# huang-yh/SelfOcc

Hardware: AMD Instinct MI355X
Metric: rendered rays/sec (6-cam 450x800, 128 samples/ray) (higher is better)
Workload: dtype f32; 1 GPU; BASELINE configs[1]: 6 cams x 450x800 rays, 128 samples/ray, volume 200x200x16; volume_channels=1, feat_storage=f32, preheat_steps=150

## Files before the change

### selfocc_amd/csrc/render_fwd.hip

```cpp
#include "render_row.h"
#include "ray_device.h"

int so_render_fwd_samples(const so_render_args &a, hipStream_t st);

namespace {

SO_DEVFN RayGeom so_pixel_ray(const so_render_args &a, int cam, int ix, int iy) {
    typedef const __attribute__((address_space(4))) float *so_const_fptr;
    const so_const_fptr M = (so_const_fptr)(a.img2lidar + cam * 16);
    float u = (float)ix * a.sx + a.ox;
    float v = (float)iy * a.sy + a.oy;
    RayGeom g;
    g.ox = M[3]; g.oy = M[7]; g.oz = M[11];
    float dx = (M[0] * u + M[1] * v) + M[2];
    float dy = (M[4] * u + M[5] * v) + M[6];
    float dz = (M[8] * u + M[9] * v) + M[10];
    g.dn = sqrtf((dx * dx + dy * dy) + dz * dz);
    g.dx = dx / g.dn; g.dy = dy / g.dn; g.dz = dz / g.dn;
    return g;
}

template <int NF, bool BF16>
SO_DEVFN void so_gather_feat(const void *__restrict__ vol, int H, int W, int D, const so_cell &c,
                             const float wk[8], float f[NF > 0 ? NF : 1]) {
// ... 781 lines not shown
        st.gh = gh; st.gw = gw; st.gd = gd;
        const int h0 = so_floor_i(gh), w0 = so_floor_i(gw), d0 = so_floor_i(gd);
        st.h0 = h0; st.w0 = w0; st.d0 = d0;
        st.cell = so_cell_index(h0, w0, d0, W, D);
    };
    auto interior = [&](const AheadStep &st) __attribute__((always_inline)) {
        return so_all3((unsigned)st.h0 < (unsigned)(H - 1), (unsigned)st.w0 < (unsigned)(W - 1), (unsigned)st.d0 < (unsigned)(D - 1));
    };
    int i_lo = S, i_hi = -1;
    {
        AheadStep p;
        const int n = min(kSureScan, S);
#pragma nounroll
        for (int k = 0; k < n; ++k) {
            place(k, p);
            if (interior(p)) { i_lo = k; break; }
        }
        if (i_lo < S) {
#pragma nounroll
            for (int k = S - 1; k >= S - n && k >= i_lo; --k) {
                place(k, p);
                if (interior(p)) { i_hi = k; break; }
            }
        }
        if (i_hi < 0) i_lo = S;
    }
    auto locate = [&](const int i, AheadStep &st, auto in_sure) __attribute__((always_inline)) {
        place(i, st);
        if constexpr (decltype(in_sure)::value) {
            st.code = __builtin_amdgcn_raw_buffer_load_b8(rb, st.cell, codes_off, 0);
        } else {
            st.all_interior = interior(st);
            st.code = 0u;
            if (st.all_interior) st.code = __builtin_amdgcn_raw_buffer_load_b8(rb, st.cell, codes_off, 0);
        }
    };
    auto near_face = [&](float fh, float fw, float fd) __attribute__((always_inline)) {
        return fmaxf(fmaxf(fabsf(fh - 0.5f), fabsf(fw - 0.5f)), fabsf(fd - 0.5f)) > 0.5f - face_m;
    };
    auto canon_cell = [&](const int i) __attribute__((always_inline)) {
        RayGeom gc = geom(so_reload_args());
        {
            unsigned ones = ~0u;
            asm volatile("" : "+s"(ones));
            const unsigned lane = __builtin_amdgcn_mbcnt_hi(ones, __builtin_amdgcn_mbcnt_lo(ones, 0u));
            const float *slot = s_dir + (wave_slot + lane);
            gc.dx = slot[0]; gc.dy = slot[256]; gc.dz = slot[512];
        }
        __builtin_amdgcn_sched_barrier(0);
        float px, py, pz;
        {
            const so_render_args ac = so_reload_args();
            const int n = ac.n_samples;
            const float b0 = so_bin(i, n);
            const float t_start = b0 * tfar + (1.0f - b0) * tnear;
            if (ac.sample_pos == SO_SAMPLE_AT_START) {
                px = gc.ox + gc.dx * t_start; py = gc.oy + gc.dy * t_start; pz = gc.oz + gc.dz * t_start;
            } else {
                const float b1 = so_bin(i + 1, n);
                const float tt = t_start + (b1 * tfar + (1.0f - b1) * tnear);
                px = gc.ox + (gc.dx * tt) / 2.0f; py = gc.oy + (gc.dy * tt) / 2.0f; pz = gc.oz + (gc.dz * tt) / 2.0f;
            }
        }
        __builtin_amdgcn_sched_barrier(0);
        float slope;
        auto axis = [](so_axis A) __attribute__((always_inline)) { A.size1 = 0.0f; return A; };
        const float gh = so_grid_coord(so_axis_m2g(axis(so_reload_args().map.h), py, slope), so_reload_args().map.h.tot_len);
        __builtin_amdgcn_sched_barrier(0);
        const float gw = so_grid_coord(so_axis_m2g(axis(so_reload_args().map.w), px, slope), so_reload_args().map.w.tot_len);
        __builtin_amdgcn_sched_barrier(0);
        const float gd = so_grid_coord(so_axis_m2g(axis(so_reload_args().map.d), pz, slope), so_reload_args().map.d.tot_len);
        return so_cell_of(gh, gw, gd);
    };

    auto step = [&](const int i, AheadStep &cur, AheadStep &nxt, auto in_sure, bool &hint) __attribute__((always_inline)) {
        constexpr bool IN_SURE = decltype(in_sure)::value;
        bool skip;
        if constexpr (IN_SURE) {
            const auto free_lanes = __builtin_amdgcn_ballot_w64((int)cur.code >= rcode);
            skip = free_lanes == __builtin_amdgcn_ballot_w64(true);
            if constexpr (kLowMode) hint = free_lanes == 0;
            locate(i + 1, nxt, in_sure);
        } else {
            skip = cur.all_interior && so_all((int)cur.code >= rcode);
            if (i + 1 < S) locate(i + 1, nxt, in_sure);
        }
        float w;
        if (skip) {
            w = kAlphaFree * T;
            T = T * ((1.0f - kAlphaFree) + 1e-7f);
        } else {
            float fh = __builtin_amdgcn_fractf(cur.gh), fw = __builtin_amdgcn_fractf(cur.gw), fd = __builtin_amdgcn_fractf(cur.gd);
            so_f32x2 p0, p1, p2, p3;
            auto gather = [&](int h0, int w0, int d0) __attribute__((always_inline)) {
                float v[8];
                so_gather_sdf_buf(rs, H, W, D, h0, w0, d0, v);
                p0 = so_f32x2{v[0], v[4]}; p1 = so_f32x2{v[1], v[5]}; p2 = so_f32x2{v[2], v[6]}; p3 = so_f32x2{v[3], v[7]};
            };
            bool moved_any = false;
            if (FACE_SAFE && __builtin_expect(__any(near_face(fh, fw, fd)), 0)) {
                int h0 = cur.h0, w0 = cur.w0, d0 = cur.d0;
                bool moved = false;
                if (near_face(fh, fw, fd)) {
                    const so_cell c = canon_cell(i);
                    moved = (c.h0 != h0) | (c.w0 != w0) | (c.d0 != d0);
                    h0 = moved ? c.h0 : h0; w0 = moved ? c.w0 : w0; d0 = moved ? c.d0 : d0;
                    fh = moved ? c.fh1 : fh; fw = moved ? c.fw1 : fw; fd = moved ? c.fd1 : fd;
                }
                moved_any = __any(moved);
                if (moved_any) gather(h0, w0, d0);
            }
            if (__builtin_expect(!moved_any, 1)) {
                if (IN_SURE || cur.all_interior) {
                    {
                        const so_f4v lo = so_bload4(rb, cur.cell * 16u, 0u), hi = so_bload4(rb, cur.cell * 16u, row_off);
                        p0 = lo.xy; p1 = lo.zw; p2 = hi.xy; p3 = hi.zw;
                    }
                } else {
                    gather(cur.h0, cur.w0, cur.d0);
                }
            }
            float sdf, dh0, gvw, gvd;
            so_trilerp_fast_pk(p0, p1, p2, p3, fh, fw, fd, sdf, dh0, gvw, gvd);
            const float cosv = fmaf(gvd, Gdd, fmaf(gvw, Gdw, dh0 * Gdh));
            const float alpha = so_alpha_fast(sdf * s2, fminf(cosv, 0.0f) * hdt_s2);
            w = alpha * T;
            T = T * ((1.0f - alpha) + 1e-7f);
        }
        const float t_mid = fmaf(cur.fi, dt, tnear + hdt);
        acc = acc + w;
        dsum = fmaf(w, t_mid, dsum);
        if (w > best_w) { best_w = w; best_t = t_mid; }
        return skip;
    };

    auto low = [&](int &i, AheadStep &st) __attribute__((always_inline)) {
        struct so_f3 { float h, w, d; };
        using so_f3r = so_f3 &;
        auto fractions = [&]() __attribute__((always_inline)) {
            return so_f3{__builtin_amdgcn_fractf(st.gh), __builtin_amdgcn_fractf(st.gw), __builtin_amdgcn_fractf(st.gd)};
        };
        so_f3 f0 = fractions(), f1;
        bool coded = false;
        bool go = i + 1 < i_hi && !(FACE_SAFE && __any(near_face(f0.h, f0.w, f0.d)));
        auto trip = [&](so_f4v &lo, so_f4v &hi, so_f4v &nlo, so_f4v &nhi, so_f3r f, so_f3r nf) __attribute__((always_inline)) {
            if constexpr (!kLowPrefetch) { lo = so_bload4(rb, st.cell * 16u, 0u); hi = so_bload4(rb, st.cell * 16u, row_off); }
            float t_mid = fmaf(st.fi, dt, tnear + hdt);
            asm volatile("" : "+v"(t_mid));
            ++i;
            place(i, st);
            if constexpr (kLowPrefetch) {
                nlo = so_bload4(rb, st.cell * 16u, 0u); nhi = so_bload4(rb, st.cell * 16u, row_off);
                __builtin_amdgcn_sched_barrier(0);
                nf = fractions();
            }
            const bool proven = __any(lo.x <= low_thr);
            float sdf, dh0, gvw, gvd;
            so_trilerp_fast_pk(lo.xy, lo.zw, hi.xy, hi.zw, f.h, f.w, f.d, sdf, dh0, gvw, gvd);
            const float cosv = fmaf(gvd, Gdd, fmaf(gvw, Gdw, dh0 * Gdh));
            float alpha = so_alpha_fast(sdf * s2, fminf(cosv, 0.0f) * hdt_s2);
            if (__builtin_expect(!proven, 0)) {
                AheadStep was;
                place(i - 1, was);
                const unsigned code = __builtin_amdgcn_raw_buffer_load_b8(rb, was.cell, codes_off, 0);
                unsigned next_cell = st.cell;
                if constexpr (kLowPrefetch) {
                    int ia = i;
                    asm volatile("" : "+s"(ia));
                    AheadStep now;
                    place(ia, now);
                    next_cell = now.cell;
                }
                st.code = __builtin_amdgcn_raw_buffer_load_b8(rb, next_cell, codes_off, 0);
                if (so_all((int)code >= rcode)) alpha = kAlphaFree;
                coded = true;
            }
            const float w = alpha * T;
            T = T * ((1.0f - alpha) + 1e-7f);
            acc = acc + w;
            dsum = fmaf(w, t_mid, dsum);
            if (w > best_w) { best_w = w; best_t = t_mid; }
            if constexpr (!kLowPrefetch) nf = fractions();
            go = !coded && !over_now() && i + 1 < i_hi && !(FACE_SAFE && __any(near_face(nf.h, nf.w, nf.d)));
        };
        so_f4v lo0, hi0, lo1, hi1;
        if constexpr (kLowPrefetch) {
            if (go) {
                lo0 = so_bload4(rb, st.cell * 16u, 0u); hi0 = so_bload4(rb, st.cell * 16u, row_off);
#pragma nounroll
                for (;;) {
                    trip(lo0, hi0, lo1, hi1, f0, f1);
                    if (!go) break;
                    trip(lo1, hi1, lo0, hi0, f1, f0);
                    if (!go) break;
                }
                int ii = i;
                asm volatile("" : "+s"(ii));
                place(ii, st);
            }
        } else {
#pragma nounroll
            while (go) trip(lo0, hi0, lo1, hi1, f0, f0);
        }
        if (over_now()) return true;
        if (!coded) st.code = __builtin_amdgcn_raw_buffer_load_b8(rb, st.cell, codes_off, 0);
        return false;
    };

    auto run = [&](int &i, AheadStep &st) __attribute__((always_inline)) {
        auto free_step = [&]() __attribute__((always_inline)) {
            const float t_mid = fmaf(st.fi, dt, tnear + hdt);
            ++i;
            place(i, st);
            st.code = __builtin_amdgcn_raw_buffer_load_b8(rb, st.cell, codes_off, 0);
            const float w = kAlphaFree * T;
            T = T * ((1.0f - kAlphaFree) + 1e-7f);
            acc = acc + w;
            dsum = fmaf(w, t_mid, dsum);
        };
        const bool kept = kSpentExit ? (__builtin_amdgcn_ballot_w64(T * 0x1p24f >= acc) & __builtin_amdgcn_ballot_w64(T >= 2e-10f)) != 0
                                     : !so_all(T < 2e-10f);
        if (S <= kRunExitFreeSteps && kept) {
            while (i < i_hi && so_all((int)st.code >= rcode)) free_step();
        } else {
            while (i < i_hi && so_all((int)st.code >= rcode)) {
                free_step();
                if (over_now()) return true;
            }
        }
        return false;
    };

    {
        constexpr std::false_type general{};
        constexpr std::true_type in_sure{};
        AheadStep A, B;
        locate(0, A, general);
        int i = 0;
        bool over = false, unused_hint = false;
        auto gen = [&](int end) __attribute__((always_inline)) {
#pragma nounroll
            while (i < end) {
                step(i, A, B, general, unused_hint);
                if (++i >= S || over_now()) { over = true; break; }
                A = B;
            }
        };
        gen(i_lo);
        if (!over) {
            while (i < i_hi) {
                const bool sa = step(i, A, B, in_sure, low_hint_a);
                ++i;
                if (over_now() || (sa && run(i, B))) { over = true; break; }
                if (i >= i_hi) { A = B; break; }
                const bool sb = step(i, B, A, in_sure, low_hint_b);
                ++i;
                if (over_now() || (sb && run(i, A))) { over = true; break; }
                if constexpr (kLowMode) {
                    if (low_hint_a && low_hint_b && low(i, A)) { over = true; break; }
                }
            }
            if (!over) { A.all_interior = true; gen(S); }
        }
    }

    const float eps32 = 1.1920928955078125e-07f;
    if (dt * inv_dn < eps32) best_t = tnear + hdt;
    float depth = dsum * so_fast_rcp(acc + 1e-10f);
    if (a.flags & SO_FLAG_DEPTH_DIV_NORM) depth = depth * inv_dn;
    if (a.depth) a.depth[ray] = depth;
    if (a.acc) a.acc[ray] = acc;
    if (a.max_depth) a.max_depth[ray] = best_t * inv_dn;
    if (a.nears) a.nears[ray] = tnear;
    if (a.fars) a.fars[ray] = tfar;
}

enum class March {
    Canonical,
    Fast,
    FastFaceSafe,
    Skip,
    SkipFaceSafe,
    CanonicalUpscale,
};
constexpr bool so_is_fast(March m) { return m == March::Fast || m == March::FastFaceSafe; }
constexpr bool so_is_skip(March m) { return m == March::Skip || m == March::SkipFaceSafe; }
constexpr bool so_face_safe(March m) { return m == March::FastFaceSafe || m == March::SkipFaceSafe; }
template <class ROW>
constexpr bool so_is_staged(March m) { return so_is_fast(m) && !ROW::BF16 && ROW::NF >= 4; }

template <class ROW, March MODE, class GeomFn>
SO_DEVFN void so_march(const so_render_args &a, int ray, GeomFn geom) {
    static_assert(!so_is_skip(MODE), "skip marcher: the kernels that take so_launch_consts");
    if constexpr (MODE == March::CanonicalUpscale) {
        so_march_exact<ROW, SO_MAP_UPSCALE>(a, ray, geom(a));
    } else if constexpr (so_is_fast(MODE)) {
        so_march_fast<ROW, false, so_face_safe(MODE)>(a, ray, geom);
    } else {
        so_march_exact<ROW, SO_MAP_LINEAR>(a, ray, geom(a));
    }
}


__global__ __launch_bounds__(256) void sdf_brickify_kernel(const float *__restrict__ vol, float *__restrict__ brick,
                                                           int H, int W, int D, so_render_args a, int with_codes,
                                                           so_launch_consts c) {
    const int h = blockIdx.x, h1 = min(h + 1, H - 1);
    const size_t n_cells = (size_t)H * W * D;
    uint8_t *codes = (uint8_t *)(brick + n_cells * 4);
    const bool quads = (D & 3) == 0 && (blockDim.x & 3) == 0;
    const float kd = c.kd.k1, kw = c.kw.k1, kh = c.kh.k1;
    for (int w = blockIdx.y * blockDim.y + threadIdx.y; w < W; w += gridDim.y * blockDim.y) {
        const int w1 = min(w + 1, W - 1);
        const float *r00 = vol + ((size_t)h * W + w) * D, *r01 = vol + ((size_t)h * W + w1) * D;
        const float *r10 = vol + ((size_t)h1 * W + w) * D, *r11 = vol + ((size_t)h1 * W + w1) * D;
        for (int d = threadIdx.x; d < D; d += blockDim.x) {
            const int d1 = min(d + 1, D - 1);
            const float v0 = r00[d], v1 = r00[d1], v2 = r01[d], v3 = r01[d1];
            const float v4 = r10[d], v5 = r10[d1], v6 = r11[d], v7 = r11[d1];
            const size_t cell = ((size_t)h * W + w) * D + d;
            ((float4 *)brick)[cell] = make_float4(v0, v4, v1, v5);
            unsigned code = 0u;
            if (with_codes) {
                const float m = fminf(fminf(fminf(v0, v1), fminf(v2, v3)), fminf(fminf(v4, v5), fminf(v6, v7)));
                const float gd = fmaxf(fmaxf(fabsf(v1 - v0), fabsf(v3 - v2)), fmaxf(fabsf(v5 - v4), fabsf(v7 - v6))) * kd;
                const float gw = fmaxf(fmaxf(fabsf(v2 - v0), fabsf(v3 - v1)), fmaxf(fabsf(v6 - v4), fabsf(v7 - v5))) * kw;
                const float gh = fmaxf(fmaxf(fabsf(v4 - v0), fabsf(v5 - v1)), fmaxf(fabsf(v6 - v2), fabsf(v7 - v3))) * kh;
                const float G = sqrtf((gd * gd + gw * gw) + gh * gh) * 1.001f + 1e-20f;
                const float slack = m - kSkipArg / so_inv_s(a);
                if (slack > 0.0f && so_inv_s(a) > 0.0f) {
                    const float allow = 2.0f * slack / G / c.skip_unit;
                    code = (unsigned)fminf(floorf(allow * 0.999f), 255.0f);
                }
            }
            if (quads) {
                const unsigned c1 = (unsigned)__builtin_amdgcn_update_dpp(0, (int)code, 0x55, 0xf, 0xf, false);
                const unsigned c2 = (unsigned)__builtin_amdgcn_update_dpp(0, (int)code, 0xaa, 0xf, 0xf, false);
                const unsigned c3 = (unsigned)__builtin_amdgcn_update_dpp(0, (int)code, 0xff, 0xf, 0xf, false);
                if ((d & 3) == 0) *(unsigned *)(codes + cell) = code | (c1 << 8) | (c2 << 16) | (c3 << 24);
            } else {
                codes[cell] = (uint8_t)code;
            }
        }
    }
}

struct TilePixel { int cam, ix, iy, wave, lane; };
SO_DEVFN TilePixel so_tile_pixel(int tiles_x, int tiles_y) {
    const int b = blockIdx.x;
    const int cam = b / (tiles_x * tiles_y);
    const int tb = b - cam * tiles_x * tiles_y;
    const int ty = tb / tiles_x, tx = tb - ty * tiles_x;
    const int wave = threadIdx.x >> 6, lane = threadIdx.x & 63;
    return {cam, tx * 16 + (wave & 1) * 8 + (lane & 7), ty * 16 + (wave >> 1) * 8 + (lane >> 3), wave, lane};
}

template <class ROW>
constexpr int so_min_blocks() { return (ROW::NB == 0 && ROW::NF >= 8) ? 2 : 1; }

template <class ROW, March MODE>
__global__ __launch_bounds__(256, so_min_blocks<ROW>()) void render_fwd_explicit(so_render_args a) {
    int ray = blockIdx.x * blockDim.x + threadIdx.x;
    if (ray >= a.n_rays) return;
    auto geom = [&](const so_render_args &a) __attribute__((always_inline)) { return so_explicit_ray(a, ray); };
    so_march<ROW, MODE>(a, ray, geom);
}

template <class ROW, March MODE>
SO_DEVFN void pixgrid_body(const so_render_args &a, int tiles_x, int tiles_y) {
    const TilePixel p = so_tile_pixel(tiles_x, tiles_y);
    const int cam = p.cam, wave = p.wave, lane = p.lane;
    int ix = p.ix, iy = p.iy;
    if constexpr (so_is_staged<ROW>(MODE)) {
        constexpr int NF = ROW::NF;
        __shared__ __attribute__((aligned(16))) float s_stage[4 * StageGeom<NF>::kWaveDwords];
        const bool real = (ix < a.nx) && (iy < a.ny);
        ix = min(ix, a.nx - 1); iy = min(iy, a.ny - 1);
        int ray = (cam * a.ny + iy) * a.nx + ix;
        auto geom = [&](const so_render_args &a) __attribute__((always_inline)) { return so_pixel_ray(a, cam, ix, iy); };
        constexpr int NSEM_LDS = NF - 3 >= 16 ? NF - 3 : 0;
        __shared__ float s_sem[NSEM_LDS > 0 ? NSEM_LDS * 256 : 1];
        so_march_fast<ROW, true, so_face_safe(MODE)>(a, ray, geom, real, s_stage + wave * StageGeom<NF>::kWaveDwords, lane,
                                                     s_sem + threadIdx.x);
    } else {
        if (ix >= a.nx || iy >= a.ny) return;
        int ray = (cam * a.ny + iy) * a.nx + ix;
        auto geom = [&](const so_render_args &a) __attribute__((always_inline)) { return so_pixel_ray(a, cam, ix, iy); };
        so_march<ROW, MODE>(a, ray, geom);
    }
}

template <class ROW, March MODE>
__global__ __launch_bounds__(256, so_min_blocks<ROW>()) void render_fwd_pixgrid(so_render_args a, int tiles_x, int tiles_y) {
    if constexpr (ROW::NB > 0) {
        const int b = blockIdx.x;
        const int cam = b / (tiles_x * tiles_y);
        const int tb = b - cam * tiles_x * tiles_y;
        const int ty = tb / tiles_x, tx = tb - ty * tiles_x;
        const int wave = threadIdx.x >> 6, lane = threadIdx.x & 63;
        const int ix = tx * 16 + (wave & 1) * 8 + (lane & 7);
        const int iy = ty * 16 + (wave >> 1) * 8 + (lane >> 3);
        if (ix >= a.nx || iy >= a.ny) return;
        const int ray = (cam * a.ny + iy) * a.nx + ix;
        so_march_exact<ROW, MODE == March::CanonicalUpscale ? SO_MAP_UPSCALE : SO_MAP_LINEAR>(a, ray, so_pixel_ray(a, cam, ix, iy));
    } else {
        pixgrid_body<ROW, MODE>(a, tiles_x, tiles_y);
    }
}

template <class ROW, March MODE>
__global__ __launch_bounds__(256, 1) void render_fwd_explicit(so_render_args a, so_launch_consts c) {
    static_assert(so_is_skip(MODE) && ROW::NF == 0 && ROW::NB == 0, "skip marcher: SDF-only launches");
    int ray = blockIdx.x * blockDim.x + threadIdx.x;
    if (ray >= a.n_rays) return;
    auto geom = [&](const so_render_args &a) __attribute__((always_inline)) { return so_explicit_ray(a, ray); };
    so_march_fast_ahead<so_face_safe(MODE)>(a, c, ray, geom);
}
#ifdef SO_NO_ROW_ORDER
constexpr bool kRowsOutermost = false;
#else
constexpr bool kRowsOutermost = true;
#endif
template <class ROW, March MODE>
__global__ __launch_bounds__(256, 1) __attribute__((amdgpu_num_sgpr(80))) void render_fwd_pixgrid(so_render_args a, so_launch_consts c) {
    static_assert(so_is_skip(MODE) && ROW::NF == 0 && ROW::NB == 0, "skip marcher: SDF-only launches");
    const int cam = kRowsOutermost ? blockIdx.y : blockIdx.z, row = kRowsOutermost ? blockIdx.z : blockIdx.y;
    const int wave = threadIdx.x >> 6, lane = threadIdx.x & 63;
    const int ix = blockIdx.x * 16 + (wave & 1) * 8 + (lane & 7), iy = row * 16 + (wave >> 1) * 8 + (lane >> 3);
    if (ix >= a.nx || iy >= a.ny) return;
    const int ray = (cam * a.ny + iy) * a.nx + ix;
    auto geom = [&](const so_render_args &a) __attribute__((always_inline)) { return so_pixel_ray(a, cam, ix, iy); };
    so_march_fast_ahead<so_face_safe(MODE)>(a, c, ray, geom);
}
bool so_skip_grid_fits(const so_render_args &a) {
    return a.ray_mode == SO_RAYS_EXPLICIT || ((a.ny + 15) / 16 <= 65535 && a.n_cams <= 65535);
}

template <class ROW, March MODE>
int launch_fwd(const so_render_args &a, hipStream_t st) {
    const int tiles_x = (a.nx + 15) / 16, tiles_y = (a.ny + 15) / 16;
    if constexpr (so_is_skip(MODE)) {
        const so_launch_consts c = so_make_launch_consts(a);
        if (a.ray_mode == SO_RAYS_EXPLICIT) {
            hipLaunchKernelGGL((render_fwd_explicit<ROW, MODE>), dim3((a.n_rays + 255) / 256), dim3(256), 0, st, a, c);
        } else {
            const dim3 grid = kRowsOutermost ? dim3(tiles_x, a.n_cams, tiles_y) : dim3(tiles_x, tiles_y, a.n_cams);
            hipLaunchKernelGGL((render_fwd_pixgrid<ROW, MODE>), grid, dim3(256), 0, st, a, c);
        }
    } else if (a.ray_mode == SO_RAYS_EXPLICIT) {
        int blocks = (a.n_rays + 255) / 256;
        hipLaunchKernelGGL((render_fwd_explicit<ROW, MODE>), dim3(blocks), dim3(256), 0, st, a);
    } else {
        int blocks = tiles_x * tiles_y * a.n_cams;
        hipLaunchKernelGGL((render_fwd_pixgrid<ROW, MODE>), dim3(blocks), dim3(256), 0, st, a, tiles_x, tiles_y);
    }
    return so_launch_status();
}

void so_launch_brickify(const so_render_args &a, hipStream_t st, int with_codes) {
    const int H = a.map.h.tot_len, W = a.map.w.tot_len, D = a.map.d.tot_len;
    int qx = 1;
    while (qx < D && qx < 256) qx *= 2;
    const int wy = 256 / qx;
    hipLaunchKernelGGL(sdf_brickify_kernel, dim3(H, min((W + wy - 1) / wy, 65535)), dim3(qx, wy), 0, st, a.sdf_vol, a.sdf_brick,
                       H, W, D, a, with_codes, so_make_launch_consts(a));
}

bool so_fast_eligible(const so_render_args &a) {
    return !(a.flags & SO_FLAG_EXACT) && a.jitter_mode == SO_JITTER_NONE && a.map.kind == SO_MAP_LINEAR &&
           a.map.h.size1 == 0.0f && a.map.w.size1 == 0.0f && a.map.d.size1 == 0.0f &&
           (long long)a.map.h.tot_len * a.map.w.tot_len < (1 << 24) && a.map.d.tot_len < (1 << 24);
}

template <class ROW, int MK>
int dispatch(const so_render_args &a, hipStream_t st) {
    if constexpr (MK == SO_MAP_UPSCALE) return launch_fwd<ROW, March::CanonicalUpscale>(a, st);
    else if constexpr (ROW::NB > 0) return launch_fwd<ROW, March::Canonical>(a, st);
    else {
        if (!so_fast_eligible(a)) return launch_fwd<ROW, March::Canonical>(a, st);
        constexpr bool CAN_SKIP = ROW::NF == 0;
        if (a.sdf_brick) so_launch_brickify(a, st, (CAN_SKIP && !(a.flags & SO_FLAG_NO_SKIP)) ? 1 : 0);
        const bool face_safe = ROW::MASKED || !(a.flags & SO_FLAG_NO_FACE_SAFE);
        if constexpr (CAN_SKIP) {
            if (a.sdf_brick && !(a.flags & (SO_FLAG_NO_SKIP | SO_FLAG_NO_AHEAD)) && so_skip_grid_fits(a))
                return face_safe ? launch_fwd<ROW, March::SkipFaceSafe>(a, st) : launch_fwd<ROW, March::Skip>(a, st);
        }
        if constexpr (!ROW::MASKED) {
            if (!face_safe) return launch_fwd<ROW, March::Fast>(a, st);
        }
        return launch_fwd<ROW, March::FastFaceSafe>(a, st);
    }
}

}

int so_validate_mapping(const so_mapping &m) {
    SO_REQUIRE(m.kind == SO_MAP_LINEAR || m.kind == SO_MAP_UPSCALE, "mapping: unknown kind %d (0 = linear, 1 = linear_upscale)",
               (int)m.kind);
    const so_axis *ax[3] = {&m.h, &m.w, &m.d};
    const so_upscale_axis *ux[3] = {&m.uh, &m.uw, &m.ud};
    for (int i = 0; i < 3; ++i) {
        SO_REQUIRE(ax[i]->tot_len >= 2, "mapping axis %d: tot_len must be >= 2", i);
        SO_REQUIRE(ax[i]->size0 > 0 && ax[i]->range0 > 0, "mapping axis %d: size0/range0 must be > 0", i);
        if (m.kind == SO_MAP_LINEAR) {
            SO_REQUIRE(ax[i]->size1 == 0 || ax[i]->range1 > 0, "mapping axis %d: range1 must be > 0", i);
        } else {
            SO_REQUIRE(ax[i]->size1 >= 1, "linear_upscale axis %d: outer cells must be >= 1 (got %g)", i, (double)ax[i]->size1);
            SO_REQUIRE(ux[i]->unit > 0 && __builtin_isfinite(ux[i]->unit), "linear_upscale axis %d: unit must be > 0 (got %g)", i,
                       (double)ux[i]->unit);
            SO_REQUIRE(ux[i]->inc > 0 && __builtin_isfinite(ux[i]->inc),
                       "linear_upscale axis %d: increase unit must be > 0 (got %g): the outer range must exceed outer * unit",
                       i, (double)ux[i]->inc);
        }
    }
    return 0;
}

namespace {
template <int MK>
__global__ __launch_bounds__(256) void meter2grid_kernel(so_mapping m, const float *__restrict__ xyz, int n, int normalize,
                                                         float *__restrict__ hwd) {
    const int i = blockIdx.x * blockDim.x + threadIdx.x;
    if (i >= n) return;
    float gh, gw, gd, sh, sw, sd;
    so_m2g<MK>(m, xyz[3 * (size_t)i], xyz[3 * (size_t)i + 1], xyz[3 * (size_t)i + 2], gh, gw, gd, sh, sw, sd);
    if (normalize) {
        gh = gh / (float)(m.h.tot_len - 1); gw = gw / (float)(m.w.tot_len - 1); gd = gd / (float)(m.d.tot_len - 1);
    }
    hwd[3 * (size_t)i] = gh; hwd[3 * (size_t)i + 1] = gw; hwd[3 * (size_t)i + 2] = gd;
}
}

extern "C" int selfocc_meter2grid(const so_mapping *map, const float *xyz, int n, int normalize, float *hwd, void *stream) {
    SO_REQUIRE(map != nullptr, "map is NULL");
    if (so_validate_mapping(*map)) return -1;
    SO_REQUIRE(n >= 0, "n must be >= 0");
    if (n == 0) return 0;
    SO_REQUIRE(xyz != nullptr && hwd != nullptr, "xyz / hwd is NULL");
    const dim3 grid((unsigned)((n + 255) / 256));
    if (map->kind == SO_MAP_UPSCALE)
        hipLaunchKernelGGL(meter2grid_kernel<SO_MAP_UPSCALE>, grid, dim3(256), 0, (hipStream_t)stream, *map, xyz, n, normalize, hwd);
    else
        hipLaunchKernelGGL(meter2grid_kernel<SO_MAP_LINEAR>, grid, dim3(256), 0, (hipStream_t)stream, *map, xyz, n, normalize, hwd);
    return so_launch_status();
}

int so_validate_render(const so_render_args &a) {
    if (so_validate_mapping(a.map)) return -1;
    SO_REQUIRE(a.sdf_vol != nullptr, "sdf_vol is NULL");
    SO_REQUIRE(a.n_samples >= 1, "n_samples must be >= 1");
    SO_REQUIRE(a.n_rays >= 0, "n_rays must be >= 0");
    SO_REQUIRE(a.n_rgb == 0 || a.n_rgb == 3, "n_rgb must be 0 or 3 (the colour outputs; sh_deg sets the coefficient count)");
    SO_REQUIRE(a.n_sem >= 0, "n_sem must be >= 0");
    SO_REQUIRE(a.n_sem == 0 || a.n_rgb == 3, "semantic channels require n_rgb == 3");
    SO_REQUIRE(a.sh_deg >= 0 && a.sh_deg <= 2, "sh_deg %d is not built (built: sh_deg 0, 1, 2)", (int)a.sh_deg);
    SO_REQUIRE(a.sh_act == SO_SH_RELU || a.sh_act == SO_SH_SIGMOID, "sh_act %d is unknown (0 = relu, 1 = sigmoid)", (int)a.sh_act);
    if (a.n_rgb + a.n_sem > 0) {
        SO_REQUIRE(a.feat_vol != nullptr, "feat_vol is NULL but n_rgb + n_sem > 0");
        SO_REQUIRE(a.feat_dtype == SO_DTYPE_F32 || a.feat_dtype == SO_DTYPE_BF16, "bad feat_dtype");
        SO_REQUIRE(a.feat_stride % 4 == 0 && a.feat_stride >= a.n_rgb + a.n_sem,
                   "feat_stride must be a multiple of 4 and >= n_rgb + n_sem");
    }
    if (so_sh_launch(a)) {
        const int n_coef = 3 * (a.sh_deg + 1) * (a.sh_deg + 1);
        SO_REQUIRE(a.n_sem == 0, "sh_deg > 0 / sh_act = sigmoid with n_sem = %d semantic channels is not built (built: n_sem = 0)",
                   (int)a.n_sem);
        SO_REQUIRE(a.feat_dtype == SO_DTYPE_F32, "sh_deg > 0 / sh_act = sigmoid with a bfloat16 feature volume is not built (built: float32)");
        SO_REQUIRE(a.feat_stride == so_sh_stride(n_coef / 3), "sh_deg = %d reads %d coefficients: feat_stride must be %d (got %d)",
                   (int)a.sh_deg, n_coef, so_sh_stride(n_coef / 3), (int)a.feat_stride);
    }
    if (a.n_sem > 0 && !so_sh_launch(a)) {
        const int stride = so_row_width(a.n_sem);
        SO_REQUIRE(a.n_sem != 1, "n_sem = 1 is not built (built: n_sem 0 and 2 .. 21): one class renders `acc`");
        SO_REQUIRE(a.n_sem <= 21, "n_sem = %d is not built (built: n_sem 0 and 2 .. 21): the binned backward record and the "
                   "32-lanes-per-sample brick kernel end at 24 channels", (int)a.n_sem);
        SO_REQUIRE(a.feat_stride == stride, "n_sem = %d semantic channels: feat_stride must be %d = 3 + n_sem rounded up to 4 (got %d)",
                   (int)a.n_sem, stride, (int)a.feat_stride);
        SO_REQUIRE(a.feat_dtype == SO_DTYPE_F32 || a.n_sem == 21, "bfloat16 feature volumes with semantic channels are built for "
                   "n_sem = 21, feat_stride = 24 only (got n_sem = %d)", (int)a.n_sem);
    }
    if (a.ray_mode == SO_RAYS_EXPLICIT) {
        SO_REQUIRE(a.n_rays == 0 || (a.origins && a.dirs), "explicit rays need origins and dirs");
    } else if (a.ray_mode == SO_RAYS_PIXEL_GRID) {
        SO_REQUIRE(a.img2lidar != nullptr, "pixel-grid rays need img2lidar");
        SO_REQUIRE(a.n_cams >= 0 && a.nx >= 0 && a.ny >= 0, "bad pixel grid");
        SO_REQUIRE((int64_t)a.n_cams * a.nx * a.ny == a.n_rays, "n_rays != n_cams * ny * nx");
    } else {
        SO_REQUIRE(false, "bad ray_mode %d", a.ray_mode);
    }
    SO_REQUIRE(a.jitter_mode >= SO_JITTER_NONE && a.jitter_mode <= SO_JITTER_EDGES, "bad jitter_mode %d", (int)a.jitter_mode);
    SO_REQUIRE(a.jitter_mode == SO_JITTER_NONE || a.t_rand, "jitter or explicit edges requested but t_rand is NULL");
    SO_REQUIRE(a.bkgd_mode != SO_BKGD_PER_RAY || a.bkgd_rays, "per-ray background but bkgd_rays is NULL");
    SO_REQUIRE(a.sample_pos == SO_SAMPLE_AT_START || a.sample_pos == SO_SAMPLE_AT_MID, "bad sample_pos");
    return 0;
}

extern "C" int selfocc_render_fwd(const so_render_args *args, void *stream) {
    SO_REQUIRE(args != nullptr, "args is NULL");
    const so_render_args &a = *args;
    if (so_validate_render(a)) return -1;
    if (a.n_rays == 0) return 0;
    hipStream_t st = (hipStream_t)stream;
    if (a.weights || a.ts || a.deltas || a.sdf || a.grad) return so_render_fwd_samples(a, st);
    return so_with_row_and_map(a, [&](auto row, auto mk) { return dispatch<decltype(row), decltype(mk)::value>(a, st); });
}
```

Baseline: 8.146 billion rays/s.

## Process two H slices per brickify thread, reusing rows via buffer loads

```diff
diff --git a/selfocc_amd/csrc/render_fwd.hip b/selfocc_amd/csrc/render_fwd.hip
--- a/selfocc_amd/csrc/render_fwd.hip
+++ b/selfocc_amd/csrc/render_fwd.hip
@@ -1107,44 +1107,71 @@
 }
 
 
+constexpr int kBrickHB = 2;
+constexpr int kBrickRecordAux = 16;
+SO_DEVFN float so_bload1(__amdgpu_buffer_rsrc_t r, unsigned voff, unsigned soff) {
+    return __builtin_bit_cast(float, __builtin_amdgcn_raw_buffer_load_b32(r, voff, soff, 0));
+}
+struct so_brick_row { float v00, v01, v10, v11; };
+SO_DEVFN so_brick_row so_brick_load_row(__amdgpu_buffer_rsrc_t rv, unsigned o00, unsigned o01, unsigned o10, unsigned o11,
+                                        unsigned row) {
+    return {so_bload1(rv, o00, row), so_bload1(rv, o01, row), so_bload1(rv, o10, row), so_bload1(rv, o11, row)};
+}
 __global__ __launch_bounds__(256) void sdf_brickify_kernel(const float *__restrict__ vol, float *__restrict__ brick,
                                                            int H, int W, int D, so_render_args a, int with_codes,
                                                            so_launch_consts c) {
-    const int h = blockIdx.x, h1 = min(h + 1, H - 1);
-    const size_t n_cells = (size_t)H * W * D;
-    uint8_t *codes = (uint8_t *)(brick + n_cells * 4);
+    typedef unsigned so_u4v __attribute__((ext_vector_type(4)));
+    const int h_lo = blockIdx.x * kBrickHB, h_hi = min(h_lo + kBrickHB, H);
+    const __amdgpu_buffer_rsrc_t rv = so_make_rsrc(vol, (size_t)c.n_cells * 4);
+    const __amdgpu_buffer_rsrc_t rb = so_make_rsrc(brick, (size_t)c.n_cells * 17);
+    const unsigned slice = (unsigned)W * (unsigned)D;
     const bool quads = (D & 3) == 0 && (blockDim.x & 3) == 0;
     const float kd = c.kd.k1, kw = c.kw.k1, kh = c.kh.k1;
+    const float inv_s = so_inv_s(a);
+    const float sat = kSkipArg / inv_s;
+    const bool can_skip = with_codes && inv_s > 0.0f;
     for (int w = blockIdx.y * blockDim.y + threadIdx.y; w < W; w += gridDim.y * blockDim.y) {
         const int w1 = min(w + 1, W - 1);
-        const float *r00 = vol + ((size_t)h * W + w) * D, *r01 = vol + ((size_t)h * W + w1) * D;
-        const float *r10 = vol + ((size_t)h1 * W + w) * D, *r11 = vol + ((size_t)h1 * W + w1) * D;
+        const unsigned c0 = __umul24((unsigned)w, (unsigned)D), c1 = __umul24((unsigned)w1, (unsigned)D);
         for (int d = threadIdx.x; d < D; d += blockDim.x) {
             const int d1 = min(d + 1, D - 1);
-            const float v0 = r00[d], v1 = r00[d1], v2 = r01[d], v3 = r01[d1];
-            const float v4 = r10[d], v5 = r10[d1], v6 = r11[d], v7 = r11[d1];
-            const size_t cell = ((size_t)h * W + w) * D + d;
-            ((float4 *)brick)[cell] = make_float4(v0, v4, v1, v5);
-            unsigned code = 0u;
-            if (with_codes) {
-                const float m = fminf(fminf(fminf(v0, v1), fminf(v2, v3)), fminf(fminf(v4, v5), fminf(v6, v7)));
-                const float gd = fmaxf(fmaxf(fabsf(v1 - v0), fabsf(v3 - v2)), fmaxf(fabsf(v5 - v4), fabsf(v7 - v6))) * kd;
-                const float gw = fmaxf(fmaxf(fabsf(v2 - v0), fabsf(v3 - v1)), fmaxf(fabsf(v6 - v4), fabsf(v7 - v5))) * kw;
-                const float gh = fmaxf(fmaxf(fabsf(v4 - v0), fabsf(v5 - v1)), fmaxf(fabsf(v6 - v2), fabsf(v7 - v3))) * kh;
-                const float G = sqrtf((gd * gd + gw * gw) + gh * gh) * 1.001f + 1e-20f;
-                const float slack = m - kSkipArg / so_inv_s(a);
-                if (slack > 0.0f && so_inv_s(a) > 0.0f) {
-                    const float allow = 2.0f * slack / G / c.skip_unit;
-                    code = (unsigned)fminf(floorf(allow * 0.999f), 255.0f);
+            const unsigned col = c0 + (unsigned)d;
+            const unsigned o00 = col * 4u, o01 = (c0 + (unsigned)d1) * 4u, o10 = (c1 + (unsigned)d) * 4u, o11 = (c1 + (unsigned)d1) * 4u;
+            so_brick_row lo = so_brick_load_row(rv, o00, o01, o10, o11, (unsigned)h_lo * slice * 4u);
+            so_brick_row hi = so_brick_load_row(rv, o00, o01, o10, o11, (unsigned)min(h_lo + 1, H - 1) * slice * 4u);
+#pragma nounroll
+            for (int h = h_lo; h < h_hi; ++h) {
+                so_brick_row nx = hi;
+                if (h + 1 < h_hi) nx = so_brick_load_row(rv, o00, o01, o10, o11, (unsigned)min(h + 2, H - 1) * slice * 4u);
+                const float v0 = lo.v00, v1 = lo.v01, v2 = lo.v10, v3 = lo.v11;
+                const float v4 = hi.v00, v5 = hi.v01, v6 = hi.v10, v7 = hi.v11;
+                const unsigned cell0 = (unsigned)h * slice;
+                const so_f4v rec = {v0, v4, v1, v5};
+                __builtin_amdgcn_raw_buffer_store_b128(__builtin_bit_cast(so_u4v, rec), rb, col * 16u, cell0 * 16u, kBrickRecordAux);
+                unsigned code = 0u;
+                if (can_skip) {
+                    const float m = fminf(fminf(fminf(v0, v1), fminf(v2, v3)), fminf(fminf(v4, v5), fminf(v6, v7)));
+                    const float gd = fmaxf(fmaxf(fabsf(v1 - v0), fabsf(v3 - v2)), fmaxf(fabsf(v5 - v4), fabsf(v7 - v6))) * kd;
+                    const float gw = fmaxf(fmaxf(fabsf(v2 - v0), fabsf(v3 - v1)), fmaxf(fabsf(v6 - v4), fabsf(v7 - v5))) * kw;
+                    const float gh = fmaxf(fmaxf(fabsf(v4 - v0), fabsf(v5 - v1)), fmaxf(fabsf(v6 - v2), fabsf(v7 - v3))) * kh;
+                    const float G = sqrtf((gd * gd + gw * gw) + gh * gh) * 1.001f + 1e-20f;
+                    const float slack = m - sat;
+                    if (slack > 0.0f) {
+                        const float allow = 2.0f * slack / G / c.skip_unit;
+                        code = (unsigned)fminf(floorf(allow * 0.999f), 255.0f);
+                    }
                 }
-            }
-            if (quads) {
-                const unsigned c1 = (unsigned)__builtin_amdgcn_update_dpp(0, (int)code, 0x55, 0xf, 0xf, false);
-                const unsigned c2 = (unsigned)__builtin_amdgcn_update_dpp(0, (int)code, 0xaa, 0xf, 0xf, false);
-                const unsigned c3 = (unsigned)__builtin_amdgcn_update_dpp(0, (int)code, 0xff, 0xf, 0xf, false);
-                if ((d & 3) == 0) *(unsigned *)(codes + cell) = code | (c1 << 8) | (c2 << 16) | (c3 << 24);
-            } else {
-                codes[cell] = (uint8_t)code;
+                if (quads) {
+                    const unsigned q1 = (unsigned)__builtin_amdgcn_update_dpp(0, (int)code, 0x55, 0xf, 0xf, false);
+                    const unsigned q2 = (unsigned)__builtin_amdgcn_update_dpp(0, (int)code, 0xaa, 0xf, 0xf, false);
+                    const unsigned q3 = (unsigned)__builtin_amdgcn_update_dpp(0, (int)code, 0xff, 0xf, 0xf, false);
+                    if ((d & 3) == 0)
+                        __builtin_amdgcn_raw_buffer_store_b32(code | (q1 << 8) | (q2 << 16) | (q3 << 24), rb, col, c.codes_off + cell0, 0);
+                } else {
+                    __builtin_amdgcn_raw_buffer_store_b8((uint8_t)code, rb, col, c.codes_off + cell0, 0);
+                }
+                lo = hi;
+                hi = nx;
             }
         }
     }
@@ -1267,14 +1294,16 @@
     int qx = 1;
     while (qx < D && qx < 256) qx *= 2;
     const int wy = 256 / qx;
-    hipLaunchKernelGGL(sdf_brickify_kernel, dim3(H, min((W + wy - 1) / wy, 65535)), dim3(qx, wy), 0, st, a.sdf_vol, a.sdf_brick,
-                       H, W, D, a, with_codes, so_make_launch_consts(a));
+    hipLaunchKernelGGL(sdf_brickify_kernel, dim3((H + kBrickHB - 1) / kBrickHB, min((W + wy - 1) / wy, 65535)), dim3(qx, wy), 0, st,
+                       a.sdf_vol, a.sdf_brick, H, W, D, a, with_codes, so_make_launch_consts(a));
 }
 
 bool so_fast_eligible(const so_render_args &a) {
+    const long long hw = (long long)a.map.h.tot_len * a.map.w.tot_len;
     return !(a.flags & SO_FLAG_EXACT) && a.jitter_mode == SO_JITTER_NONE && a.map.kind == SO_MAP_LINEAR &&
            a.map.h.size1 == 0.0f && a.map.w.size1 == 0.0f && a.map.d.size1 == 0.0f &&
-           (long long)a.map.h.tot_len * a.map.w.tot_len < (1 << 24) && a.map.d.tot_len < (1 << 24);
+           hw < (1 << 24) && a.map.d.tot_len < (1 << 24) &&
+           (!a.sdf_brick || hw * a.map.d.tot_len * 17 <= 0xfffffffcll);
 }
 
 template <class ROW, int MK>
```

Result: no change. 8.197 billion rays/s (median of 6 runs) (+0.6%).
